# menyifang/MIMO

Hardware: NVIDIA H100
Metric: frames/sec @ 512x512x24f, 20 DDIM steps (higher is better)
Workload: dtype fp16

## Files before the change

### mimo_b200/csrc/attn_spatial.cu

```cuda
#include <cuda_runtime.h>

#include "../../include/mimo_b200.h"
#include "attn_common.h"
#include "host_util.h"
#include "ptx.cuh"
#include "wgmma.cuh"

namespace mimo {

template <int DP>
struct AttnCfg {
  static constexpr int NCH = (DP + 63) / 64;
  static constexpr int NWG = DP >= 160 ? 1 : 2;
  static constexpr int QROWS = 64 * NWG;
  static constexpr int kThreads = 128 * NWG + 32;
  static constexpr int kQChunk = QROWS * 128;
  static constexpr int kQBytes = NCH * kQChunk;
  static constexpr int kKVStageBytes = 2 * NCH * kChunkBytes;
  static constexpr int kFit = (227 * 1024 - 1024 - 256 - kQBytes) / kKVStageBytes;
  static constexpr int KVST = kFit < 4 ? kFit : 4;
  static constexpr bool kLook = NWG == 2 && KVST >= 2 && DP <= 80;
  static constexpr int kSmemBytes = kQBytes + KVST * kKVStageBytes + 1024 + 256;
  static_assert(KVST >= 1, "K/V tile does not fit");
};

template <bool kMask, bool kBf16>
__device__ __forceinline__ void softmax_tile(float (&s)[BKV / 2], int valid, int q2, float scale_log2, float (&m)[2],
                                             float (&l)[2], float (&alpha)[2], uint32_t (&pa)[BKV / 16][4]) {
  float mx[2] = {-INFINITY, -INFINITY};
#pragma unroll
  for (int jn = 0; jn < BKV / 8; ++jn)
#pragma unroll
    for (int e = 0; e < 4; ++e) {
      if (!kMask || 8 * jn + q2 + (e & 1) < valid)
        mx[e >> 1] = fmaxf(mx[e >> 1], s[4 * jn + e]);
      else
        s[4 * jn + e] = -INFINITY;
    }
  float m_new[2];
#pragma unroll
  for (int r = 0; r < 2; ++r) {
    mx[r] = fmaxf(mx[r], __shfl_xor_sync(0xffffffffu, mx[r], 1));
    mx[r] = fmaxf(mx[r], __shfl_xor_sync(0xffffffffu, mx[r], 2));
    m_new[r] = fmaxf(m[r], mx[r] * scale_log2);
    alpha[r] = ex2_ftz(m[r] - m_new[r]);
  }
  float rowsum[2] = {0.f, 0.f};
#pragma unroll
  for (int kk = 0; kk < BKV / 16; ++kk)
#pragma unroll
    for (int i = 0; i < 4; ++i) {
      const int e = 8 * kk + 2 * i;
      const int r = i & 1;
      const float p0 = ex2_ftz(fmaf(s[e], scale_log2, -m_new[r]));
      const float p1 = ex2_ftz(fmaf(s[e + 1], scale_log2, -m_new[r]));
      rowsum[r] += p0 + p1;
      pa[kk][i] = Cvt<kBf16>::pack(p0, p1);
    }
#pragma unroll
  for (int r = 0; r < 2; ++r) {
    l[r] = l[r] * alpha[r] + rowsum[r];
    m[r] = m_new[r];
  }
}

template <bool kBf16>
__device__ __forceinline__ void softmax_step(float (&s)[BKV / 2], int valid, int q2, float scale_log2, float (&m)[2],
                                             float (&l)[2], float (&alpha)[2], uint32_t (&pa)[BKV / 16][4]) {
  if (valid < BKV)
    softmax_tile<true, kBf16>(s, valid, q2, scale_log2, m, l, alpha, pa);
  else
    softmax_tile<false, kBf16>(s, valid, q2, scale_log2, m, l, alpha, pa);
}

template <int DP, bool kBf16>
__global__ void __launch_bounds__(AttnCfg<DP>::kThreads, 1)
attn_spatial_kernel(const __grid_constant__ CUtensorMap tmQ, const __grid_constant__ CUtensorMap tmK,
                    const __grid_constant__ CUtensorMap tmV, const __grid_constant__ CUtensorMap tmBK,
                    const __grid_constant__ CUtensorMap tmBV, AttnArgs a) {
  using Cfg = AttnCfg<DP>;
  using C = Cvt<kBf16>;
  constexpr int NCH = Cfg::NCH, KVST = Cfg::KVST, kProd = 4 * Cfg::NWG;
  extern __shared__ uint8_t smem_raw[];
  uint8_t* smem = reinterpret_cast<uint8_t*>((reinterpret_cast<uintptr_t>(smem_raw) + 1023) & ~uintptr_t(1023));
  uint8_t* sQ = smem;
  uint8_t* sKV = sQ + Cfg::kQBytes;
  uint64_t* bars = reinterpret_cast<uint64_t*>(sKV + KVST * Cfg::kKVStageBytes);
  uint64_t* q_full = bars;
  uint64_t* kv_full = bars + 1;
  uint64_t* kv_empty = kv_full + KVST;

  const int warp = __shfl_sync(0xffffffffu, threadIdx.x >> 5, 0);
  const int lane = threadIdx.x & 31;
  const int q_tile = blockIdx.x;
  const int h = blockIdx.y;
  const int n = blockIdx.z;
  pdl_launch_dependents();
  pdl_wait();
  const int bidx = __shfl_sync(0xffffffffu, a.bank_index ? a.bank_index[n] : -1, 0);
  const int T = a.n_self_tiles + (bidx >= 0 ? a.n_bank_tiles : 0);

  if (warp == kProd && lane == 0) {
    tma_prefetch_desc(&tmQ);
    tma_prefetch_desc(&tmK);
    tma_prefetch_desc(&tmV);
    if (bidx >= 0) {
      tma_prefetch_desc(&tmBK);
      tma_prefetch_desc(&tmBV);
    }
  }
  if (warp == kProd && lane == 1) {
    mbar_init(q_full, 1);
    for (int s = 0; s < KVST; ++s) {
      mbar_init(&kv_full[s], 1);
      mbar_init(&kv_empty[s], kProd);
    }
    fence_mbar_init();
  }
  __syncthreads();

  if (warp == kProd) {
    if (lane != 0) return;
    mbar_expect_tx(q_full, Cfg::kQBytes);
#pragma unroll
    for (int ch = 0; ch < NCH; ++ch) tma_load_4d(sQ + ch * Cfg::kQChunk, &tmQ, q_full, ch * 64, h, q_tile * Cfg::QROWS, n);
    for (int j = 0; j < T; ++j) {
      const int stage = j % KVST;
      const uint32_t phase = (j / KVST) & 1u;
      mbar_wait(&kv_empty[stage], phase ^ 1u);
      uint8_t* sk = sKV + stage * Cfg::kKVStageBytes;
      uint8_t* sv = sk + NCH * kChunkBytes;
      mbar_expect_tx(&kv_full[stage], Cfg::kKVStageBytes);
      const bool bank = j >= a.n_self_tiles;
      const int row0 = (bank ? j - a.n_self_tiles : j) * BKV;
      const int img = bank ? bidx : n;
      const CUtensorMap* mk = bank ? &tmBK : &tmK;
      const CUtensorMap* mv = bank ? &tmBV : &tmV;
#pragma unroll
      for (int ch = 0; ch < NCH; ++ch) {
        tma_load_4d(sk + ch * kChunkBytes, mk, &kv_full[stage], ch * 64, h, row0, img);
        tma_load_4d(sv + ch * kChunkBytes, mv, &kv_full[stage], ch * 64, h, row0, img);
      }
    }
    return;
  }
  const int wg = warp >> 2;
  const int rbase = wg * 64 + (warp & 3) * 16 + (lane >> 2);
  const int q2 = (lane & 3) * 2;
  const uint32_t q_addr = smem_u32(sQ) + wg * (64 * 128);
  const float scale_log2 = a.scale_log2;
  auto tile_valid = [&](int j) {
    const bool bank = j >= a.n_self_tiles;
    const int valid = (bank ? a.lb : a.lq) - (bank ? j - a.n_self_tiles : j) * BKV;
    return valid < BKV ? valid : BKV;
  };
  auto kv_addr = [&](int j) { return smem_u32(sKV + (j % KVST) * Cfg::kKVStageBytes); };
  auto wait_kv = [&](int j) { mbar_wait(&kv_full[j % KVST], (j / KVST) & 1u); };
  auto issue_s = [&](float (&s)[BKV / 2], uint32_t k_addr) {
#pragma unroll
    for (int ks = 0; ks < DP / 16; ++ks) {
      const uint32_t off = (ks & 3) * 32;
      Wgmma<BKV, kBf16>::ss(s, make_smem_desc_sw128(q_addr + (ks >> 2) * Cfg::kQChunk + off, 16, 1024),
                            make_smem_desc_sw128(k_addr + (ks >> 2) * kChunkBytes + off, 16, 1024), ks != 0 ? 1u : 0u);
    }
  };
  float o[DP / 2];
  auto issue_pv = [&](const uint32_t (&pa)[BKV / 16][4], uint32_t v_addr, bool first) {
#pragma unroll
    for (int kk = 0; kk < BKV / 16; ++kk) {
      Wgmma<DP, kBf16>::rs(o, pa[kk], make_smem_desc_sw128(v_addr + kk * 2048, kChunkBytes, 1024),
                           (!first || kk != 0) ? 1u : 0u);
    }
  };
  auto release = [&](int j) {
    if (lane == 0) mbar_arrive(&kv_empty[j % KVST]);
  };
  float m[2] = {-INFINITY, -INFINITY}, l[2] = {0.f, 0.f}, alpha[2];
  float s[BKV / 2];
  uint32_t pa[BKV / 16][4];
  mbar_wait(q_full, 0);

  if constexpr (Cfg::kLook) {
    const int bar_mine = 1 + wg, bar_other = 2 - wg;
    if (wg == 1) bar_arrive(bar_other, 256);
    wait_kv(0);
    bar_sync(bar_mine, 256);
    wgmma_fence();
    issue_s(s, kv_addr(0));
    wgmma_commit();
    bar_arrive(bar_other, 256);
    wgmma_wait<0>();
    reg_fence(s);
    softmax_step<kBf16>(s, tile_valid(0), q2, scale_log2, m, l, alpha, pa);
    for (int j = 0; j + 1 < T; ++j) {
      wait_kv(j + 1);
      bar_sync(bar_mine, 256);
      wgmma_fence();
      issue_s(s, kv_addr(j + 1));
      wgmma_commit();
      issue_pv(pa, kv_addr(j) + NCH * kChunkBytes, j == 0);
      wgmma_commit();
      bar_arrive(bar_other, 256);
      uint32_t pn[BKV / 16][4];
      wgmma_wait<1>();
      reg_fence(s);
      softmax_step<kBf16>(s, tile_valid(j + 1), q2, scale_log2, m, l, alpha, pn);
      wgmma_wait<0>();
      reg_fence(o);
      release(j);
#pragma unroll
      for (int i = 0; i < DP / 2; ++i) o[i] *= alpha[(i >> 1) & 1];
#pragma unroll
      for (int kk = 0; kk < BKV / 16; ++kk)
#pragma unroll
        for (int i = 0; i < 4; ++i) pa[kk][i] = __byte_perm(pa[kk][i], pn[kk][i], 0x7654);
    }
    bar_sync(bar_mine, 256);
    wgmma_fence();
    issue_pv(pa, kv_addr(T - 1) + NCH * kChunkBytes, T == 1);
    wgmma_commit();
    if (wg == 0) bar_arrive(bar_other, 256);
    wgmma_wait<0>();
    reg_fence(o);
    release(T - 1);
  } else {
    for (int j = 0; j < T; ++j) {
      wait_kv(j);
      wgmma_fence();
      issue_s(s, kv_addr(j));
      wgmma_commit();
      wgmma_wait<0>();
      reg_fence(s);
      softmax_step<kBf16>(s, tile_valid(j), q2, scale_log2, m, l, alpha, pa);
      if (j > 0) {
#pragma unroll
        for (int i = 0; i < DP / 2; ++i) o[i] *= alpha[(i >> 1) & 1];
      }
      wgmma_fence();
      issue_pv(pa, kv_addr(j) + NCH * kChunkBytes, j == 0);
      wgmma_commit();
      wgmma_wait<0>();
      reg_fence(o);
      release(j);
    }
  }
#pragma unroll
  for (int r = 0; r < 2; ++r) {
    l[r] += __shfl_xor_sync(0xffffffffu, l[r], 1);
    l[r] += __shfl_xor_sync(0xffffffffu, l[r], 2);
    const float inv_l = 1.0f / l[r];
    const int qrow = q_tile * Cfg::QROWS + rbase + 8 * r;
    if (qrow < a.lq) {
      typename C::T* orow =
          static_cast<typename C::T*>(a.out) + (static_cast<long long>(n) * a.lq + qrow) * a.ld_out + h * a.d;
#pragma unroll
      for (int jn = 0; jn < DP / 8; ++jn)
        if (8 * jn + q2 < a.d)
          *reinterpret_cast<uint32_t*>(orow + 8 * jn + q2) = C::pack(o[4 * jn + 2 * r] * inv_l, o[4 * jn + 2 * r + 1] * inv_l);
    }
  }
}

static int attn_tmap(CUtensorMap* m, int dtype, const void* base, int d, int heads, int len, int nimg, long long ld,
                     uint32_t rows = BKV);

template <int DP, bool kBf16>
static int launch_attn(const mimo_attn_params* p, const CUtensorMap& k, const CUtensorMap& v, const CUtensorMap& bk,
                       const CUtensorMap& bv, const AttnArgs& a, cudaStream_t st) {
  using Cfg = AttnCfg<DP>;
  auto kern = attn_spatial_kernel<DP, kBf16>;
  static bool attr_done = false;
  if (!attr_done) {
    cudaError_t e = cudaFuncSetAttribute(kern, cudaFuncAttributeMaxDynamicSharedMemorySize, Cfg::kSmemBytes);
    if (e != cudaSuccess) return set_cuda_error("cudaFuncSetAttribute(attn)", e);
    attr_done = true;
  }
  CUtensorMap q;
  if (int rc = attn_tmap(&q, p->dtype, p->q, p->d, p->heads, p->lq, p->n, p->ld_qkv, Cfg::QROWS)) return rc;
  const dim3 grid((p->lq + Cfg::QROWS - 1) / Cfg::QROWS, p->heads, p->n);
  cudaError_t e = launch_k(kern, grid, dim3(Cfg::kThreads), Cfg::kSmemBytes, st, q, k, v, bk, bv, a);
  if (e == cudaSuccess) e = cudaGetLastError();
  if (e != cudaSuccess) return set_cuda_error("attn launch", e);
  return MIMO_OK;
}

static int attn_tmap(CUtensorMap* m, int dtype, const void* base, int d, int heads, int len, int nimg, long long ld,
                     uint32_t rows) {
  const uint64_t dims[4] = {static_cast<uint64_t>(d), static_cast<uint64_t>(heads), static_cast<uint64_t>(len),
                            static_cast<uint64_t>(nimg)};
  const uint64_t str[3] = {static_cast<uint64_t>(d) * 2, static_cast<uint64_t>(ld) * 2,
                           static_cast<uint64_t>(len) * ld * 2};
  const uint32_t box[4] = {64, 1, rows, 1};
  return encode_tmap(m, dtype, 4, base, dims, str, box);
}

}

using namespace mimo;

extern "C" int mimo_attn_spatial(const mimo_attn_params* p, void* stream) {
  if (!p || !p->q || !p->k || !p->v || !p->out) return set_error(MIMO_ERR_ARG, "mimo_attn_spatial: null pointer");
  if (p->n <= 0 || p->lq <= 0 || p->heads <= 0 || p->d <= 0 || (p->d % 8) || p->d > 192 || (p->ld_qkv % 8) ||
      (p->ld_out % 8))
    return set_error(MIMO_ERR_ARG, "mimo_attn_spatial: need d % 8 == 0, d <= 192, leading dims % 8 == 0");
  const bool has_bank = p->bank_index && p->bank_k && p->bank_v && p->lb > 0;
  if (has_bank && (p->ld_bank % 8)) return set_error(MIMO_ERR_ARG, "mimo_attn_spatial: ld_bank % 8 != 0");
  if (int rc = ensure_device()) return rc;

  AttnArgs a;
  a.lq = p->lq;
  a.lb = has_bank ? p->lb : 0;
  a.heads = p->heads;
  a.d = p->d;
  a.dp = (p->d + 15) / 16 * 16;
  a.n_self_tiles = (p->lq + BKV - 1) / BKV;
  a.n_bank_tiles = has_bank ? (p->lb + BKV - 1) / BKV : 0;
  a.scale_log2 = p->scale * 1.4426950408889634f;
  a.bank_index = has_bank ? p->bank_index : nullptr;
  a.out = p->out;
  a.ld_out = p->ld_out;

  CUtensorMap tk, tv, tbk, tbv;
  if (int rc = attn_tmap(&tk, p->dtype, p->k, p->d, p->heads, p->lq, p->n, p->ld_qkv)) return rc;
  if (int rc = attn_tmap(&tv, p->dtype, p->v, p->d, p->heads, p->lq, p->n, p->ld_qkv)) return rc;
  if (has_bank) {
    const int nb = p->nb > 0 ? p->nb : 1;
    if (int rc = attn_tmap(&tbk, p->dtype, p->bank_k, p->d, p->heads, p->lb, nb, p->ld_bank)) return rc;
    if (int rc = attn_tmap(&tbv, p->dtype, p->bank_v, p->d, p->heads, p->lb, nb, p->ld_bank)) return rc;
  } else {
    tbk = tk;
    tbv = tv;
  }
  cudaStream_t st = static_cast<cudaStream_t>(stream);
  switch (a.dp) {
#define MIMO_ATTN_DP(DP) \
  case DP:               \
    return p->dtype == MIMO_BF16 ? launch_attn<DP, true>(p, tk, tv, tbk, tbv, a, st) \
                                 : launch_attn<DP, false>(p, tk, tv, tbk, tbv, a, st);
    MIMO_ATTN_DP(16) MIMO_ATTN_DP(32) MIMO_ATTN_DP(48) MIMO_ATTN_DP(64) MIMO_ATTN_DP(80) MIMO_ATTN_DP(96)
    MIMO_ATTN_DP(112) MIMO_ATTN_DP(128) MIMO_ATTN_DP(144) MIMO_ATTN_DP(160) MIMO_ATTN_DP(176) MIMO_ATTN_DP(192)
#undef MIMO_ATTN_DP
  }
  return set_error(MIMO_ERR_ARG, "mimo_attn_spatial: unsupported head dim");
}
```

Measured before the change: 8.173.

## Use four consumer warpgroups with inline TMA production for head dim 48

For head dim 48 the spatial attention kernel now runs four warpgroups (256 query rows per CTA) and drops the dedicated producer warp. Thread 0 of the first consumer warp issues the Q and K/V TMA loads itself, refilling ring stages opportunistically with mbarrier test and blocking only when a needed tile is not yet loaded. This is meant to amortise each K/V tile load over more query rows and to remove the extra producer warp, at the cost of fewer CTAs, the serial non-lookahead loop, and possible stalls in warp 0 while it produces. A compile-time phase timer using clock64 stamps is also added but stays disabled by default.

```diff
diff --git a/mimo_b200/csrc/attn_spatial.cu b/mimo_b200/csrc/attn_spatial.cu
--- a/mimo_b200/csrc/attn_spatial.cu
+++ b/mimo_b200/csrc/attn_spatial.cu
@@ -11,9 +11,10 @@
 template <int DP>
 struct AttnCfg {
   static constexpr int NCH = (DP + 63) / 64;
-  static constexpr int NWG = DP >= 160 ? 1 : 2;
+  static constexpr bool kWide = DP == 48;
+  static constexpr int NWG = DP >= 160 ? 1 : (kWide ? 4 : 2);
   static constexpr int QROWS = 64 * NWG;
-  static constexpr int kThreads = 128 * NWG + 32;
+  static constexpr int kThreads = 128 * NWG + (kWide ? 0 : 32);
   static constexpr int kQChunk = QROWS * 128;
   static constexpr int kQBytes = NCH * kQChunk;
   static constexpr int kKVStageBytes = 2 * NCH * kChunkBytes;
@@ -73,6 +74,13 @@
     softmax_tile<false, kBf16>(s, valid, q2, scale_log2, m, l, alpha, pa);
 }
 
+#ifdef MIMO_ATTN_PHASE_TIMER
+constexpr int kPhaseTiles = 128;
+constexpr int kPhaseWords = 2 + 4 * kPhaseTiles;
+__device__ long long* g_phase_buf;
+__device__ int g_phase_slots;
+#endif
+
 template <int DP, bool kBf16>
 __global__ void __launch_bounds__(AttnCfg<DP>::kThreads, 1)
 attn_spatial_kernel(const __grid_constant__ CUtensorMap tmQ, const __grid_constant__ CUtensorMap tmK,
@@ -81,6 +89,10 @@
   using Cfg = AttnCfg<DP>;
   using C = Cvt<kBf16>;
   constexpr int NCH = Cfg::NCH, KVST = Cfg::KVST, kProd = 4 * Cfg::NWG;
+  constexpr int kTmaWarp = Cfg::kWide ? 0 : kProd;
+#ifdef MIMO_ATTN_PHASE_TIMER
+  const long long t_entry = clock64();
+#endif
   extern __shared__ uint8_t smem_raw[];
   uint8_t* smem = reinterpret_cast<uint8_t*>((reinterpret_cast<uintptr_t>(smem_raw) + 1023) & ~uintptr_t(1023));
   uint8_t* sQ = smem;
@@ -100,7 +112,7 @@
   const int bidx = __shfl_sync(0xffffffffu, a.bank_index ? a.bank_index[n] : -1, 0);
   const int T = a.n_self_tiles + (bidx >= 0 ? a.n_bank_tiles : 0);
 
-  if (warp == kProd && lane == 0) {
+  if (warp == kTmaWarp && lane == 0) {
     tma_prefetch_desc(&tmQ);
     tma_prefetch_desc(&tmK);
     tma_prefetch_desc(&tmV);
@@ -109,7 +121,7 @@
       tma_prefetch_desc(&tmBV);
     }
   }
-  if (warp == kProd && lane == 1) {
+  if (warp == kTmaWarp && lane == 1) {
     mbar_init(q_full, 1);
     for (int s = 0; s < KVST; ++s) {
       mbar_init(&kv_full[s], 1);
@@ -119,36 +131,70 @@
   }
   __syncthreads();
 
-  if (warp == kProd) {
+  auto load_q = [&]() {
+    mbar_expect_tx(q_full, Cfg::kQBytes);
+#pragma unroll
+    for (int ch = 0; ch < NCH; ++ch) tma_load_4d(sQ + ch * Cfg::kQChunk, &tmQ, q_full, ch * 64, h, q_tile * Cfg::QROWS, n);
+  };
+  auto load_kv = [&](int j) {
+    const int stage = j % KVST;
+    uint8_t* sk = sKV + stage * Cfg::kKVStageBytes;
+    uint8_t* sv = sk + NCH * kChunkBytes;
+    mbar_expect_tx(&kv_full[stage], Cfg::kKVStageBytes);
+    const bool bank = j >= a.n_self_tiles;
+    const int row0 = (bank ? j - a.n_self_tiles : j) * BKV;
+    const int img = bank ? bidx : n;
+    const CUtensorMap* mk = bank ? &tmBK : &tmK;
+    const CUtensorMap* mv = bank ? &tmBV : &tmV;
+#pragma unroll
+    for (int ch = 0; ch < NCH; ++ch) {
+      tma_load_4d(sk + ch * kChunkBytes, mk, &kv_full[stage], ch * 64, h, row0, img);
+      tma_load_4d(sv + ch * kChunkBytes, mv, &kv_full[stage], ch * 64, h, row0, img);
+    }
+  };
+  auto empty_phase = [&](int j) { return ((j / KVST) & 1u) ^ 1u; };
+  if (!Cfg::kWide && warp >= kProd) {
     if (lane != 0) return;
-    mbar_expect_tx(q_full, Cfg::kQBytes);
-#pragma unroll
-    for (int ch = 0; ch < NCH; ++ch) tma_load_4d(sQ + ch * Cfg::kQChunk, &tmQ, q_full, ch * 64, h, q_tile * Cfg::QROWS, n);
+    load_q();
     for (int j = 0; j < T; ++j) {
-      const int stage = j % KVST;
-      const uint32_t phase = (j / KVST) & 1u;
-      mbar_wait(&kv_empty[stage], phase ^ 1u);
-      uint8_t* sk = sKV + stage * Cfg::kKVStageBytes;
-      uint8_t* sv = sk + NCH * kChunkBytes;
-      mbar_expect_tx(&kv_full[stage], Cfg::kKVStageBytes);
-      const bool bank = j >= a.n_self_tiles;
-      const int row0 = (bank ? j - a.n_self_tiles : j) * BKV;
-      const int img = bank ? bidx : n;
-      const CUtensorMap* mk = bank ? &tmBK : &tmK;
-      const CUtensorMap* mv = bank ? &tmBV : &tmV;
-#pragma unroll
-      for (int ch = 0; ch < NCH; ++ch) {
-        tma_load_4d(sk + ch * kChunkBytes, mk, &kv_full[stage], ch * 64, h, row0, img);
-        tma_load_4d(sv + ch * kChunkBytes, mv, &kv_full[stage], ch * 64, h, row0, img);
+      mbar_wait(&kv_empty[j % KVST], empty_phase(j));
+      load_kv(j);
+    }
+    return;
+  }
+  const bool tma_thread = Cfg::kWide && threadIdx.x == 0;
+  int next_load = 0;
+  auto produce = [&](int need) {
+    while (next_load < T) {
+      uint64_t* e = &kv_empty[next_load % KVST];
+      if (next_load >= KVST) {
+        if (next_load <= need)
+          mbar_wait(e, empty_phase(next_load));
+        else if (!mbar_test(e, empty_phase(next_load)))
+          break;
       }
-    }
-    return;
+      load_kv(next_load++);
+    }
+  };
+  if (tma_thread) {
+    load_q();
+    produce(0);
   }
   const int wg = warp >> 2;
   const int rbase = wg * 64 + (warp & 3) * 16 + (lane >> 2);
   const int q2 = (lane & 3) * 2;
   const uint32_t q_addr = smem_u32(sQ) + wg * (64 * 128);
   const float scale_log2 = a.scale_log2;
+#ifdef MIMO_ATTN_PHASE_TIMER
+  long long* const ph = (q_tile == 0 && h == 0 && n < g_phase_slots && (warp & 3) == 0 && lane == 0)
+                            ? g_phase_buf + (n * 4 + wg) * kPhaseWords : nullptr;
+  if (ph) ph[0] = t_entry;
+  auto stamp = [&](int j, int k) {
+    if (ph && j < kPhaseTiles) ph[2 + 4 * j + k] = clock64();
+  };
+#else
+  auto stamp = [](int, int) {};
+#endif
   auto tile_valid = [&](int j) {
     const bool bank = j >= a.n_self_tiles;
     const int valid = (bank ? a.lb : a.lq) - (bank ? j - a.n_self_tiles : j) * BKV;
@@ -185,16 +231,20 @@
     if (wg == 1) bar_arrive(bar_other, 256);
     wait_kv(0);
     bar_sync(bar_mine, 256);
+    stamp(0, 0);
     wgmma_fence();
     issue_s(s, kv_addr(0));
     wgmma_commit();
     bar_arrive(bar_other, 256);
     wgmma_wait<0>();
     reg_fence(s);
+    stamp(0, 1);
     softmax_step<kBf16>(s, tile_valid(0), q2, scale_log2, m, l, alpha, pa);
+    stamp(0, 2);
     for (int j = 0; j + 1 < T; ++j) {
       wait_kv(j + 1);
       bar_sync(bar_mine, 256);
+      stamp(j + 1, 0);
       wgmma_fence();
       issue_s(s, kv_addr(j + 1));
       wgmma_commit();
@@ -204,9 +254,12 @@
       uint32_t pn[BKV / 16][4];
       wgmma_wait<1>();
       reg_fence(s);
+      stamp(j + 1, 1);
       softmax_step<kBf16>(s, tile_valid(j + 1), q2, scale_log2, m, l, alpha, pn);
+      stamp(j + 1, 2);
       wgmma_wait<0>();
       reg_fence(o);
+      stamp(j, 3);
       release(j);
 #pragma unroll
       for (int i = 0; i < DP / 2; ++i) o[i] *= alpha[(i >> 1) & 1];
@@ -222,16 +275,22 @@
     if (wg == 0) bar_arrive(bar_other, 256);
     wgmma_wait<0>();
     reg_fence(o);
+    stamp(T - 1, 3);
     release(T - 1);
   } else {
     for (int j = 0; j < T; ++j) {
+      if (tma_thread) produce(j);
+      __syncwarp();
       wait_kv(j);
+      stamp(j, 0);
       wgmma_fence();
       issue_s(s, kv_addr(j));
       wgmma_commit();
       wgmma_wait<0>();
       reg_fence(s);
+      stamp(j, 1);
       softmax_step<kBf16>(s, tile_valid(j), q2, scale_log2, m, l, alpha, pa);
+      stamp(j, 2);
       if (j > 0) {
 #pragma unroll
         for (int i = 0; i < DP / 2; ++i) o[i] *= alpha[(i >> 1) & 1];
@@ -241,6 +300,7 @@
       wgmma_commit();
       wgmma_wait<0>();
       reg_fence(o);
+      stamp(j, 3);
       release(j);
     }
   }
@@ -259,6 +319,9 @@
           *reinterpret_cast<uint32_t*>(orow + 8 * jn + q2) = C::pack(o[4 * jn + 2 * r] * inv_l, o[4 * jn + 2 * r + 1] * inv_l);
     }
   }
+#ifdef MIMO_ATTN_PHASE_TIMER
+  if (ph) ph[1] = clock64();
+#endif
 }
 
 static int attn_tmap(CUtensorMap* m, int dtype, const void* base, int d, int heads, int len, int nimg, long long ld,
@@ -297,6 +360,14 @@
 }
 
 using namespace mimo;
+
+#ifdef MIMO_ATTN_PHASE_TIMER
+extern "C" int mimo_attn_phase_timer(long long* buf, int slots) {
+  cudaError_t e = cudaMemcpyToSymbol(g_phase_buf, &buf, sizeof(buf));
+  if (e == cudaSuccess) e = cudaMemcpyToSymbol(g_phase_slots, &slots, sizeof(slots));
+  return e == cudaSuccess ? MIMO_OK : set_cuda_error("mimo_attn_phase_timer", e);
+}
+#endif
 
 extern "C" int mimo_attn_spatial(const mimo_attn_params* p, void* stream) {
   if (!p || !p->q || !p->k || !p->v || !p->out) return set_error(MIMO_ERR_ARG, "mimo_attn_spatial: null pointer");
```

Measured after the change: 8.282 (median of 6 runs). 1.3% higher.
